# DISCOWER/fault-tolerant-mpc

Hardware: AMD Instinct MI355X
Metric: MPC QP steps/s (whole node) at N=20, 8 thrusters, batch 65536 (higher is better)
Workload: dtype f32

## Files before the change

fault-tolerant-mpc_amd/csrc/ftmpc_solve.hip:

```cpp
#include <hip/hip_runtime.h>

#include <type_traits>

#include "ftmpc_common.h"

namespace ftmpc {

namespace {

typedef float f32x4 __attribute__((ext_vector_type(4)));
typedef float f32x2 __attribute__((ext_vector_type(2)));

__device__ __forceinline__ void wave_lds_fence() { asm volatile("" ::: "memory"); }
__device__ __forceinline__ void wave_global_fence() { asm volatile("s_waitcnt vmcnt(0)" ::: "memory"); }
__device__ __forceinline__ int tidx(int I, int J) { return (I * (I + 1)) / 2 + J; }

__device__ __forceinline__ float readlane_f(float x, int l) {
    return __builtin_bit_cast(float, __builtin_amdgcn_readlane(__builtin_bit_cast(int, x), l));
}
struct OpAdd { static __device__ __forceinline__ float f(float a, float b) { return a + b; } };
struct OpMin { static __device__ __forceinline__ float f(float a, float b) { return fminf(a, b); } };
struct OpMax { static __device__ __forceinline__ float f(float a, float b) { return fmaxf(a, b); } };
template <class Op>
__device__ __forceinline__ float wave_reduce(float x) {
// ... 388 lines not shown
        {
            const f32x4 wj = Wof(J);
            float y0 = wj.x * r, y1 = wj.y * r, y2 = wj.z * r, y3 = wj.w * r;
            row_sum16x4(y0, y1, y2, y3);
            Y[J] = f32x4{y0, y1, y2, y3};
        }
#pragma unroll
        for (int I = J + 1; I < NB; ++I) {
            const f32x4& t = T[tidx(I, J)];
            p[I] += f32x2{t.x, t.y} * f32x2{Y[J].x, Y[J].y};
            p[I] += f32x2{t.z, t.w} * f32x2{Y[J].z, Y[J].w};
        }
    }
    wave_lds_fence();
    f32x2 a0[NB], a1[NB];
#pragma unroll
    for (int J = 0; J < NB; ++J) a0[J] = a1[J] = f32x2{0.f, 0.f};
    const int lb = lane_now();
    const int li_b = lb & 15, lq_b = lb >> 4;
#pragma unroll
    for (int J = NB - 1; J >= 0; --J) {
        f32x4 r = Y[J];
        if (J < NB - 1) {
            float s0 = a0[J].x, s1 = a0[J].y, s2 = a1[J].x, s3 = a1[J].y;
            row_sum16x4(s0, s1, s2, s3);
            r -= f32x4{s0, s1, s2, s3};
        }
        const f32x4 wb = Wof(J);
        const f32x2 d2 = f32x2{wb.x, wb.y} * f32x2{r.x, r.y} + f32x2{wb.z, wb.w} * f32x2{r.z, r.w};
        const float xr = quad_sum(d2.x + d2.y);
        if (lq_b == 0) xv[16 * J + li_b] = xr;
        const f32x2 xx = {xr, xr};
#pragma unroll
        for (int K = 0; K < J; ++K) {
            const f32x4& t = T[tidx(J, K)];
            a0[K] += f32x2{t.x, t.y} * xx;
            a1[K] += f32x2{t.z, t.w} * xx;
        }
    }
    wave_lds_fence();
}

__host__ __device__ constexpr int aoff(int r, int c) {
    constexpr int ZERO = REC_STRIDE, ONE = REC_STRIDE + 1, DT = REC_STRIDE + 2;
    if (r >= 13) return ZERO;
    const int kind = r < 3 ? 0 : (r < 6 ? 1 : (r < 9 ? 2 : 3));
    const int a = r < 3 ? r : (r < 6 ? r - 3 : (r < 9 ? r - 6 : r - 9));
    if (c < 3) return (kind == 0 && c == a) ? ONE : ZERO;
    if (c < 6) return (kind == 0 && c - 3 == a) ? DT : ((kind == 1 && c - 3 == a) ? ONE : ZERO);
    if (c < 9) {
        const int j = c - 6;
        return kind == 0 ? REC_APW + 3 * a + j : (kind == 1 ? REC_AVW + 3 * a + j : (kind == 2 ? REC_AWW + 3 * a + j : REC_AQW + 3 * a + j));
    }
    if (c < 13) {
        const int j = c - 9;
        return kind == 0 ? REC_APQ + 4 * a + j : (kind == 1 ? REC_AVQ + 4 * a + j : (kind == 2 ? ZERO : REC_AQQ + 4 * a + j));
    }
    if (c < 16) {
        const int j = c - 13;
        return kind == 0 ? REC_BPF + 3 * a + j : (kind == 1 ? REC_BVF + 3 * a + j : ZERO);
    }
    const int j = c - 16;
    return kind == 0 ? REC_BPT + 3 * a + j : (kind == 1 ? REC_BVT + 3 * a + j : (kind == 2 ? REC_BWT + 3 * a + j : REC_BQT + 3 * a + j));
}
struct AoffTable {
    unsigned char v[16][20];
};
constexpr AoffTable make_aoff_table() {
    AoffTable t{};
    for (int r = 0; r < 16; ++r)
        for (int c = 0; c < 20; ++c) t.v[r][c] = (unsigned char)((c < 19) ? aoff(r, c) : REC_STRIDE);
    return t;
}
__device__ const AoffTable k_aoff = make_aoff_table();
typedef double f64x4 __attribute__((ext_vector_type(4)));
__device__ __forceinline__ f64x4 mfma_d(double a, double b, f64x4 c) {
    return __builtin_amdgcn_mfma_f64_16x16x4f64(a, b, c, 0, 0, 0);
}

typedef __attribute__((address_space(3))) double lds_f64;
typedef __attribute__((address_space(3))) const float lds_cf32;
typedef __attribute__((address_space(1))) double glb_f64;
typedef __attribute__((address_space(1))) const double glb_cf64;
template <class SPtr, int GOFF = 160>
__device__ __noinline__ void struct_grad(const DeviceConsts& C, glb_cf64* recg, lds_f64* recd, lds_cf32* s_Da,
                                            lds_cf32* dnat, SPtr sS, glb_f64* gout, int na, int lane) {
    constexpr int ZERO = REC_STRIDE;
    const int N = C.N;
    const int m = lane & 15, q = lane >> 4;
    int offX[4], offG[2], offAT[4], offBT[4];
#pragma unroll
    for (int s4 = 0; s4 < 4; ++s4) {
        const int k = 4 * s4 + q;
        offX[s4] = (k < 13) ? k_aoff.v[m][k] : ZERO;
        offAT[s4] = (k < 13 && m < 13) ? k_aoff.v[k][m] : ZERO;
        offBT[s4] = (k < 13 && m < 6) ? k_aoff.v[k][13 + m] : ZERO;
    }
#pragma unroll
    for (int s4 = 0; s4 < 2; ++s4) offG[s4] = (4 * s4 + q < 6) ? k_aoff.v[m][13 + 4 * s4 + q] : ZERO;
    if (lane == 0) {
        recd[REC_STRIDE] = 0.0;
        recd[REC_STRIDE + 1] = 1.0;
        recd[REC_STRIDE + 2] = C.dt;
    }
    double qrow[4], rrow[2], da_op[2];
#pragma unroll
    for (int i = 0; i < 4; ++i) qrow[i] = (q + 4 * i < 9) ? C.Q[q + 4 * i] : 0.0;
#pragma unroll
    for (int i = 0; i < 2; ++i) {
        rrow[i] = (q + 4 * i < 6) ? C.R[q + 4 * i] : 0.0;
        da_op[i] = (q + 4 * i < 6) ? (double)s_Da[(q + 4 * i) * MAX_NT + m] : 0.0;
    }
    double pa[4];
#pragma unroll
    for (int s4 = 0; s4 < 4; ++s4) pa[s4] = (m < 9 && 4 * s4 + q < 9) ? C.P[9 * m + 4 * s4 + q] : 0.0;
    const f64x4 zero = {0.0, 0.0, 0.0, 0.0};
    glb_f64* genS = gout + GOFF;
    for (int t = lane; t < N * 8; t += 64) {
        const int k = t >> 3, g = t & 7;
        double acc = 0.0;
        if (g < 6)
            for (int a = 0; a < na; ++a) acc += (double)s_Da[g * MAX_NT + a] * (double)dnat[k * na + a];
        genS[t] = acc;
    }
    __threadfence_block();
    wave_global_fence();
    const int g1 = (q + 4 < 6) ? q + 4 : 7;
    double pf[4][3], pg[4][2];
    const int w2 = (lane + 128 < REC_STRIDE) ? lane + 128 : REC_STRIDE - 1;
    const int d2 = (lane + 128 < REC_STRIDE) ? lane + 128 : REC_STRIDE + 3;
    auto issue = [&](auto SL, int kk) {
        constexpr int sl = decltype(SL)::value;
        glb_cf64* r = recg + (int64_t)kk * REC_STRIDE;
        pf[sl][0] = r[lane];
        pf[sl][1] = r[lane + 64];
        pf[sl][2] = r[w2];
        pg[sl][0] = genS[kk * 8 + q];
        pg[sl][1] = genS[kk * 8 + g1];
    };
    auto stage_to_lds = [&](auto SL) {
        constexpr int sl = decltype(SL)::value;
        recd[lane] = pf[sl][0];
        recd[lane + 64] = pf[sl][1];
        recd[d2] = pf[sl][2];
    };
    using S0 = std::integral_constant<int, 0>;
    using S1 = std::integral_constant<int, 1>;
    using S2 = std::integral_constant<int, 2>;
    using S3 = std::integral_constant<int, 3>;
    f64x4 dc = zero;
    auto fwd = [&](auto SL, int k) {
        constexpr int sl = decltype(SL)::value;
        wave_lds_fence();
        stage_to_lds(SL);
        const double g0 = pg[sl][0], g1v = pg[sl][1];
        issue(SL, (k + 4 < N) ? k + 4 : N - 1);
        wave_lds_fence();
        f64x4 nx = zero, ny = zero;
        nx = mfma_d(recd[offX[0]], dc.x, nx);
        ny = mfma_d(recd[offX[1]], dc.y, ny);
        nx = mfma_d(recd[offX[2]], dc.z, nx);
        ny = mfma_d(recd[offX[3]], dc.w, ny);
        nx = mfma_d(recd[offG[0]], g0, nx);
        ny = mfma_d(recd[offG[1]], g1v, ny);
        dc = nx + ny;
        f64x4 t = zero;
        if (k + 1 == N) {
#pragma unroll
            for (int s4 = 0; s4 < 4; ++s4) t = mfma_d(pa[s4], dc[s4], t);
        } else {
#pragma unroll
            for (int i = 0; i < 3; ++i) t[i] = qrow[i] * dc[i];
        }
        if (m == 0) {
            SPtr srow = sS + (k + 1) * 9;
            srow[q] = recd[REC_WE + q] + t.x;
            srow[q + 4] = recd[REC_WE + q + 4] + t.y;
            if (q == 0) srow[8] = recd[REC_WE + 8] + t.z;
        }
    };
    const int N4 = N & ~3;
    issue(S0{}, 0);
    issue(S1{}, (1 < N) ? 1 : 0);
    issue(S2{}, (2 < N) ? 2 : 0);
    issue(S3{}, (3 < N) ? 3 : 0);
    for (int k = 0; k < N4; k += 4) {
        fwd(S0{}, k);
        fwd(S1{}, k + 1);
        fwd(S2{}, k + 2);
        fwd(S3{}, k + 3);
    }
    for (int k = N4; k < N; ++k) {
        issue(S0{}, k);
        fwd(S0{}, k);
    }
    wave_global_fence();
    f64x4 lam = zero;
    auto adj = [&](auto SL, int k) {
        constexpr int sl = decltype(SL)::value;
        wave_lds_fence();
        stage_to_lds(SL);
        const double g0 = pg[sl][0], g1v = pg[sl][1];
        issue(SL, (k - 4 >= 0) ? k - 4 : 0);
        wave_lds_fence();
        if (k == N - 1) {
            lam.x = sS[N * 9 + q];
            lam.y = sS[N * 9 + q + 4];
            lam.z = (q == 0) ? sS[N * 9 + 8] : 0.0;
            lam.w = 0.0;
        }
        f64x4 z = zero, zb = zero;
        z = mfma_d(recd[offBT[0]], lam.x, z);
        zb = mfma_d(recd[offBT[1]], lam.y, zb);
        z = mfma_d(recd[offBT[2]], lam.z, z);
        zb = mfma_d(recd[offBT[3]], lam.w, zb);
        z += zb;
        const double z0 = z.x + recd[REC_RUT + q] + rrow[0] * g0;
        const double z1 = (q + 4 < 6) ? z.y + recd[REC_RUT + q + 4] + rrow[1] * g1v : 0.0;
        f64x4 ga = zero;
        ga = mfma_d(da_op[0], z0, ga);
        ga = mfma_d(da_op[1], z1, ga);
        if (m == 0) {
#pragma unroll
            for (int i = 0; i < 4; ++i)
                if (q + 4 * i < na) gout[k * na + q + 4 * i] = 2.0 * ga[i];
        }
        if (k > 0) {
            f64x4 nl = zero, nm = zero;
            nl = mfma_d(recd[offAT[0]], lam.x, nl);
            nm = mfma_d(recd[offAT[1]], lam.y, nm);
            nl = mfma_d(recd[offAT[2]], lam.z, nl);
            nm = mfma_d(recd[offAT[3]], lam.w, nm);
            nl += nm;
            lam.x = nl.x + sS[k * 9 + q];
            lam.y = nl.y + sS[k * 9 + q + 4];
            lam.z = nl.z + ((q == 0) ? sS[k * 9 + 8] : 0.0);
            lam.w = nl.w;
        }
    };
    issue(S0{}, N - 1);
    issue(S1{}, (N - 2 >= 0) ? N - 2 : 0);
    issue(S2{}, (N - 3 >= 0) ? N - 3 : 0);
    issue(S3{}, (N - 4 >= 0) ? N - 4 : 0);
    int ka = N - 1;
    for (; ka >= 3; ka -= 4) {
        adj(S0{}, ka);
        adj(S1{}, ka - 1);
        adj(S2{}, ka - 2);
        adj(S3{}, ka - 3);
    }
    for (; ka >= 0; --ka) {
        issue(S0{}, ka);
        adj(S0{}, ka);
    }
    __threadfence_block();
    wave_global_fence();
}

__host__ __device__ constexpr int tile_row(int r) { return r < 9 ? 4 * (r % 3) + r / 3 : (r < 12 ? 12 + (r - 9) : 3); }
constexpr int DENSE_DUMP = 256 + 128;
constexpr int DENSE_WORDS = 400;
constexpr int dense_blk(int w, int base, int ncol, int rowc, int colc, bool isB) {
    const int a = (w - base) / ncol, c = (w - base) % ncol;
    return isB ? 256 + 8 * tile_row(rowc + a) + (colc + c) : 16 * tile_row(rowc + a) + tile_row(colc + c);
}
constexpr int dense_pos(int w) {
    if (w < REC_APQ) return dense_blk(w, REC_APW, 3, 0, 6, false);
    if (w < REC_AVW) return dense_blk(w, REC_APQ, 4, 0, 9, false);
    if (w < REC_AVQ) return dense_blk(w, REC_AVW, 3, 3, 6, false);
    if (w < REC_AWW) return dense_blk(w, REC_AVQ, 4, 3, 9, false);
    if (w < REC_AQW) return dense_blk(w, REC_AWW, 3, 6, 6, false);
    if (w < REC_AQQ) return dense_blk(w, REC_AQW, 3, 9, 6, false);
    if (w < REC_BPF) return dense_blk(w, REC_AQQ, 4, 9, 9, false);
    if (w < REC_BPT) return dense_blk(w, REC_BPF, 3, 0, 0, true);
    if (w < REC_BVF) return dense_blk(w, REC_BPT, 3, 0, 3, true);
    if (w < REC_BVT) return dense_blk(w, REC_BVF, 3, 3, 0, true);
    if (w < REC_BWT) return dense_blk(w, REC_BVT, 3, 3, 3, true);
    if (w < REC_BQT) return dense_blk(w, REC_BWT, 3, 6, 3, true);
    if (w < REC_WE) return dense_blk(w, REC_BQT, 3, 9, 3, true);
    return DENSE_DUMP;
}
struct DensePosTable {
    unsigned short v[REC_STRIDE];
};
constexpr DensePosTable make_dense_pos() {
    DensePosTable t{};
    for (int w = 0; w < REC_STRIDE; ++w) t.v[w] = (unsigned short)dense_pos(w);
    return t;
}
__device__ const DensePosTable k_dense_pos = make_dense_pos();
constexpr bool dense_pos_ok() {
    bool used[DENSE_WORDS] = {};
    for (int a = 0; a < 3; ++a) {
        used[16 * tile_row(a) + tile_row(a)] = true;
        used[16 * tile_row(a) + tile_row(3 + a)] = true;
        used[16 * tile_row(3 + a) + tile_row(3 + a)] = true;
    }
    for (int w = 0; w < REC_STRIDE; ++w) {
        const int p = dense_pos(w);
        if (w >= REC_WE) {
            if (p != DENSE_DUMP) return false;
            continue;
        }
        if (p < 0 || p >= DENSE_DUMP || used[p]) return false;
        used[p] = true;
    }
    return true;
}
static_assert(dense_pos_ok(), "stage-record scatter table is inconsistent");
constexpr bool tile_row_ok() {
    bool seen[16] = {};
    for (int r = 0; r < 13; ++r) {
        const int t = tile_row(r);
        if (t < 0 || t > 15 || seen[t]) return false;
        seen[t] = true;
        if (r < 9 && ((t & 3) > 2 || (t >> 2) > 2)) return false;
    }
    return true;
}
static_assert(tile_row_ok(), "state-component permutation of the sensitivity tiles is inconsistent");

}

#ifndef FTMPC_F32_MU_POLISH
#define FTMPC_F32_MU_POLISH 1e-5f
#endif
#ifndef FTMPC_F32_REFINE_AT_POLISH
#define FTMPC_F32_REFINE_AT_POLISH 1
#endif
#ifndef FTMPC_F32_REGRAD_DD
#define FTMPC_F32_REGRAD_DD 2e-4f
#endif
#ifndef FTMPC_F32_PW0
#define FTMPC_F32_PW0 1e3f
#endif
#ifndef FTMPC_F32_OCC
#define FTMPC_F32_OCC 2
#endif
template <int NB>
__global__ void __launch_bounds__(64) __attribute__((amdgpu_waves_per_eu((NB == 8) ? FTMPC_F32_OCC : 1, (NB == 8) ? FTMPC_F32_OCC : 1))) ftmpc_solve_f32_kernel(const DeviceConsts C, const SolveParams P) {
    using SH = Shape<NB>;
    constexpr int NPAD = SH::NPAD, NV = SH::NV, NTILES = SH::NTILES;
    constexpr int NLDS = (NB == 8) ? ((FTMPC_F32_OCC > 1) ? 0 : NTILES) : (NB == 9 ? 36 : 35);
    constexpr bool OCC2 = (NB == 8) && (FTMPC_F32_OCC > 1);
    constexpr int BUILD_WORDS = 2 * DENSE_WORDS + 256;
    __shared__ __attribute__((aligned(16))) float tiles[(NLDS * 256 > BUILD_WORDS) ? NLDS * 256 : BUILD_WORDS];
    __shared__ __attribute__((aligned(16))) float recbuf[2 * REC_STRIDE + 8];
    __shared__ __attribute__((aligned(16))) float work[SH::WORK + SH::SEXTRA];
    __shared__ __attribute__((aligned(16))) float s_Da[6 * MAX_NT];
    __shared__ unsigned char s_stg[NPAD], s_thr[NPAD];
    __shared__ int s_act[MAX_NT];
    __shared__ __attribute__((aligned(16))) float wlds[OCC2 ? NB * 256 : 4];
    float* const dense = tiles;
    float* const xvp = work;
    float* const dvp = work + NPAD;

    const int lane = threadIdx.x;
    const int li = lane & 15, lq = lane >> 4;
    const int N = C.N, NT = C.NT;
    TileStore<NLDS> htiles;
    htiles.p = tiles;
    htiles.bind(P.hscratch + (int64_t)blockIdx.x * P.tile_words + slot_tile_off_words(C.N));
    const float rho = (float)C.rho;
    const float mu_stop = (float)C.mu_stop;
    float Rf[6];
#pragma unroll
    for (int g = 0; g < 6; ++g) Rf[g] = (float)C.R[g];

    auto pull = [&]() {
        int i = 0;
        if (lane == 0) i = atomicAdd(P.qhead, 1);
        return i;
    };
    const int qn = *P.qcount;
    int qnext = pull();
    for (;;) {
        const int qi = __builtin_amdgcn_readfirstlane(qnext);
        if (qi >= qn) break;
        const int64_t inst = P.qlist[qi];
        qnext = pull();
        STAMP_DECL;
        STAMP_START();
        wave_lds_fence();
        double ub_l = 0.0;
        if (lane < NT) ub_l = P.ub[inst * NT + lane];
        const unsigned long long amask = __ballot(lane < NT && ub_l > 0.0);
        const int na = __popcll(amask);
        const int n = N * na;
        const int nb = (n + 15) >> 4;
        const int npad = nb * 16;
        (void)npad;
        if (na == 0 || nb > NB) {
            if (lane < NT) P.out_u0[inst * NT + lane] = 0.0;
            if (P.out_U)
                for (int i = lane; i < N * NT; i += 64) P.out_U[inst * N * NT + i] = 0.0;
            if (lane == 0) {
                if (P.status) P.status[inst] = (na == 0) ? 0 : 2;
                if (P.iters) P.iters[inst] = 0;
            }
            continue;
        }
        const int nbr = NB;
        const int npadr = 16 * nbr;
        const int myrank = __popcll(amask & ((1ull << lane) - 1ull));
        if (lane < NT && ub_l > 0.0) s_act[myrank] = lane;
        wave_lds_fence();
        if (lane < na) {
#pragma unroll
            for (int g = 0; g < 6; ++g) s_Da[g * MAX_NT + lane] = (float)C.D[g * MAX_NT + s_act[lane]];
        }
        for (int e = lane; e < npadr; e += 64) {
            const int s = e / na;
            s_stg[e] = (unsigned char)(e < n ? s : 255);
            s_thr[e] = (unsigned char)(e < n ? e - s * na : 255);
        }
        typedef double f64x4_t __attribute__((ext_vector_type(4)));
        const double* recg = reinterpret_cast<const double*>(P.rec) + inst * (int64_t)N * REC_STRIDE;
        f64x4_t pre64 = {0.0, 0.0, 0.0, 0.0};
        if (lane < REC_STRIDE / 4) pre64 = *reinterpret_cast<const f64x4_t*>(recg + 4 * lane);
        int dpos[4] = {DENSE_DUMP, DENSE_DUMP, DENSE_DUMP, DENSE_DUMP};
        {
            int w0 = 4 * lane;
            asm volatile("" : "+v"(w0));
            if (lane < REC_STRIDE / 4) {
                const ushort4 t = *reinterpret_cast<const ushort4*>(&k_dense_pos.v[w0]);
                dpos[0] = t.x;
                dpos[1] = t.y;
                dpos[2] = t.z;
                dpos[3] = t.w;
            }
        }
        for (int i = lane; i < 2 * DENSE_WORDS + 256; i += 64) dense[i] = 0.f;
        wave_lds_fence();
        if (lane < 6) {
            const int a = lane % 3, isv = lane / 3;
#pragma unroll
            for (int bsel = 0; bsel < 2; ++bsel) {
                float* dd = dense + bsel * DENSE_WORDS;
                dd[16 * tile_row(3 * isv + a) + tile_row(3 * isv + a)] = 1.f;
                if (!isv) dd[16 * tile_row(a) + tile_row(3 + a)] = (float)C.dt;
            }
        }
        for (int i = lane; i < 81; i += 64) {
            const int r = i / 9, c = i - 9 * r;
            if (c >= r) dense[2 * DENSE_WORDS + 16 * tile_row(r) + tile_row(c)] = (float)C.LPt[i];
        }
        wave_lds_fence();
        const f32x4 lp4 = lds4(dense + 2 * DENSE_WORDS + 16 * li + 4 * lq);

        int kcol[NV], acol[NV];
        float ubar[NV], ubv[NV], gacc[NV];
#pragma unroll
        for (int v = 0; v < NV; ++v) {
            const int e = v * 64 + lane;
            kcol[v] = (e < npadr) ? s_stg[e] : 255;
            acol[v] = (e < npadr) ? s_thr[e] : 255;
            ubar[v] = 0.f;
            ubv[v] = 1.f;
            gacc[v] = 0.f;
            if (kcol[v] != 255) {
                const int t = s_act[acol[v]];
                ubv[v] = (float)P.ub[inst * NT + t];
                if (P.warmU) {
                    const float wv = (float)P.warmU[(inst * N + kcol[v]) * NT + t];
                    ubar[v] = fminf(fmaxf(wv, 0.f), ubv[v]);
                }
            }
        }
        int kX[OCC2 ? 1 : NB];
        float DaB[OCC2 ? 1 : NB][2];
        f32x4 G[NB];
        float gpart[NB];
#pragma unroll
        for (int X = 0; X < NB; ++X) {
            if constexpr (!OCC2) {
                kX[X] = s_stg[16 * X + li];
                const int ax = s_thr[16 * X + li];
                DaB[X][0] = (ax != 255) ? s_Da[lq * MAX_NT + ax] : 0.f;
                DaB[X][1] = (ax != 255 && lq < 2) ? s_Da[(4 + lq) * MAX_NT + ax] : 0.f;
            }
            G[X] = (f32x4){0.f, 0.f, 0.f, 0.f};
            gpart[X] = 0.f;
        }
        float esc[3];
#pragma unroll
        for (int s3 = 0; s3 < 3; ++s3) esc[s3] = (lq < 3) ? (OCC2 ? 2.f * (float)C.Q[3 * s3 + lq] : (float)C.sq2Q[3 * s3 + lq]) : 0.f;
        f32x4 acc[NTILES];
#pragma unroll
        for (int t = 0; t < NTILES; ++t) acc[t] = (f32x4){0.f, 0.f, 0.f, 0.f};

        float* const mtab = work;
        auto finish_tile = [&](int I, int J) {
            const int lane = lane_now();
            const int li = lane & 15, lq = lane >> 4;
            f32x4 h = acc[(I * (I + 1)) / 2 + J];
            if (J >= I - 1) {
#pragma unroll
                for (int rr = 0; rr < 4; ++rr) {
                    const int e1 = (I == J) ? 16 * I + 4 * lq + rr : 16 * I + li;
                    const int e2 = (I == J) ? 16 * J + li : 16 * J + 4 * lq + rr;
                    const int s1 = s_stg[e1], a1 = s_thr[e1];
                    const int s2 = s_stg[e2], a2 = s_thr[e2];
                    float add = (s1 != 255 && s1 == s2) ? mtab[((a1 & (MAX_NT - 1)) << 4) | (a2 & (MAX_NT - 1))] : 0.f;
                    if (s1 == 255 && e1 == e2) add = 1.f;
                    h[rr] += add;
                }
            }
            htiles.st((I * (I + 1)) / 2 + J, lane, -h);
        };

        STAMP(0);
        auto stage = [&](int k, auto TERM) {
            constexpr bool terminal = decltype(TERM)::value;
            const int lane = lane_now();
            const int li = lane & 15, lq = lane >> 4;
            float* rb = recbuf + (k & 1) * REC_STRIDE;
            float* dd = dense + (k & 1) * DENSE_WORDS;
            if (lane < REC_STRIDE / 4) {
                const f32x4 pre = {(float)pre64.x, (float)pre64.y, (float)pre64.z, (float)pre64.w};
                *reinterpret_cast<f32x4*>(rb + 4 * lane) = pre;
                dd[dpos[0]] = pre.x;
                dd[dpos[1]] = pre.y;
                dd[dpos[2]] = pre.z;
                dd[dpos[3]] = pre.w;
                if (!terminal) pre64 = *reinterpret_cast<const f64x4_t*>(recg + (k + 1) * REC_STRIDE + 4 * lane);
            }
            wave_lds_fence();
            const f32x4 a4 = lds4(dd + 16 * li + 4 * lq);
            const float b0 = dd[256 + 8 * li + lq], b1 = dd[256 + 8 * li + 4 + lq];
            float we[3];
#pragma unroll
            for (int s3 = 0; s3 < 3; ++s3) we[s3] = (lq < 3) ? rb[REC_WE + 3 * s3 + lq] : 0.f;
            const float rut0 = rb[REC_RUT + lq], rut1 = (lq < 2) ? rb[REC_RUT + 4 + lq] : 0.f;
            const int Imax = ((k + 1) * na - 1) >> 4;
            const int Xnew = (k * na) >> 4;
            float E[NB][3];
            const f32x4 zero4 = {0.f, 0.f, 0.f, 0.f};
#pragma unroll
            for (int X = 0; X < NB; ++X)
                if (X <= Imax) {
                    f32x4 o = zero4;
                    if (X >= Xnew) {
                        float d0, d1;
                        if constexpr (OCC2) {
                            const int ax = *(lds_vu8*)&s_thr[16 * X + li];
                            const bool mine = (*(lds_vu8*)&s_stg[16 * X + li] == k);
                            d0 = mine ? s_Da[lq * MAX_NT + (ax & (MAX_NT - 1))] : 0.f;
                            d1 = (mine && lq < 2) ? s_Da[(4 + lq) * MAX_NT + (ax & (MAX_NT - 1))] : 0.f;
                        } else {
                            const bool mine = (kX[X] == k);
                            d0 = mine ? DaB[X][0] : 0.f;
                            d1 = mine ? DaB[X][1] : 0.f;
                        }
                        o = mfma4(b0, d0, o);
                        o = mfma4(b1, d1, o);
                        gpart[X] += d0 * rut0 + d1 * rut1;
                    }
                    o = mfma4(a4.x, G[X].x, o);
                    o = mfma4(a4.y, G[X].y, o);
                    o = mfma4(a4.z, G[X].z, o);
                    o = mfma4(a4.w, G[X].w, o);
                    G[X] = o;
                }
#pragma unroll
            for (int X = 0; X < NB; ++X)
                if (X <= Imax) {
                    gpart[X] += we[0] * G[X].x + we[1] * G[X].y + we[2] * G[X].z;
                    if (!terminal) {
                        if constexpr (!OCC2) {
                            E[X][0] = esc[0] * G[X].x;
                            E[X][1] = esc[1] * G[X].y;
                            E[X][2] = esc[2] * G[X].z;
                        }
                    } else {
                        f32x4 o = zero4;
                        o = mfma4(lp4.x, G[X].x, o);
                        o = mfma4(lp4.y, G[X].y, o);
                        o = mfma4(lp4.z, G[X].z, o);
                        o = mfma4(lp4.w, G[X].w, o);
                        E[X][0] = o.x;
                        E[X][1] = o.y;
                        E[X][2] = o.z;
                    }
                }
            STAMP(1);
#pragma unroll
            for (int I = 0; I < NB; ++I)
                if (I <= Imax) {
                    float eI[3] = {0.f, 0.f, 0.f};
                    if constexpr (OCC2 && !terminal) {
                        eI[0] = esc[0] * G[I].x;
                        eI[1] = esc[1] * G[I].y;
                        eI[2] = esc[2] * G[I].z;
                    }
#pragma unroll
                    for (int J = 0; J <= I; ++J) {
                        if constexpr (OCC2 && !terminal) {
                            acc[(I * (I + 1)) / 2 + J] = mfma4(G[J].x, eI[0], acc[(I * (I + 1)) / 2 + J]);
                            acc[(I * (I + 1)) / 2 + J] = mfma4(G[J].y, eI[1], acc[(I * (I + 1)) / 2 + J]);
                            acc[(I * (I + 1)) / 2 + J] = mfma4(G[J].z, eI[2], acc[(I * (I + 1)) / 2 + J]);
                        } else {
#pragma unroll
                        for (int s3 = 0; s3 < 3; ++s3) acc[(I * (I + 1)) / 2 + J] = mfma4(E[J][s3], E[I][s3], acc[(I * (I + 1)) / 2 + J]);
                        }
                        if constexpr (terminal) finish_tile(I, J);
                    }
                }
            STAMP(2);
        };
        for (int k = 0; k + 1 < N; ++k) stage(k, std::false_type{});
        for (int t = lane; t < MAX_NT * MAX_NT; t += 64) {
            const int a1 = t >> 4, a2 = t & (MAX_NT - 1);
            float m = 0.f;
            if (a1 < na && a2 < na) {
#pragma unroll
                for (int g = 0; g < 6; ++g) m += s_Da[g * MAX_NT + a1] * Rf[g] * s_Da[g * MAX_NT + a2];
                if (a1 == a2) m += rho;
            }
            mtab[t] = 2.f * m;
        }
        wave_lds_fence();
        stage(N - 1, std::true_type{});
#pragma unroll
        for (int I = 0; I < NB; ++I)
            if (I > ((N * na - 1) >> 4)) {
#pragma unroll
                for (int J = 0; J <= I; ++J) finish_tile(I, J);
            }
        {
            float qs[NB];
#pragma unroll
            for (int X = 0; X < NB; ++X) qs[X] = quad_sum(gpart[X]);
#pragma unroll
            for (int v = 0; v < NV; ++v) {
                float t = 0.f;
#pragma unroll
                for (int j = 0; j < 4; ++j)
                    if (4 * v + j < NB) t = (lq == j) ? qs[4 * v + j] : t;
                gacc[v] += t;
            }
        }
        wave_lds_fence();

        float gv[NV], lo[NV], hi[NV], sl[NV], su[NV], zl[NV], zu[NV], grad[NV];
        bool valid[NV];
#pragma unroll
        for (int v = 0; v < NV; ++v) {
            valid[v] = kcol[v] != 255;
            gv[v] = valid[v] ? 2.f * (gacc[v] + rho * ubar[v]) : 0.f;
            lo[v] = -ubar[v];
            hi[v] = ubv[v] - ubar[v];
            sl[v] = su[v] = 0.5f * ubv[v];
        }
        if (P.dbg_inst == inst) {
#pragma unroll
            for (int I = 0; I < NB; ++I)
                if (I < nbr) {
#pragma unroll
                    for (int J = 0; J <= I; ++J) {
                        const f32x4 ht = htiles.ld((I * (I + 1)) / 2 + J, lane);
#pragma unroll
                        for (int rr = 0; rr < 4; ++rr) {
                            const int e1 = (I == J) ? 16 * I + 4 * lq + rr : 16 * I + li;
                            const int e2 = (I == J) ? 16 * J + li : 16 * J + 4 * lq + rr;
                            const float h = -ht[rr];
                            if (I != J || e1 >= e2) {
                                P.dbg_H[(int64_t)e1 * npadr + e2] = h;
                                P.dbg_H[(int64_t)e2 * npadr + e1] = h;
                            }
                        }
                    }
                }
#pragma unroll
            for (int v = 0; v < NV; ++v) {
                const int e = v * 64 + lane;
                if (e < npadr) {
                    P.dbg_vec[e] = gv[v];
                    P.dbg_vec[npadr + e] = lo[v];
                    P.dbg_vec[2 * npadr + e] = hi[v];
                }
            }
            if (lane == 0) {
                P.dbg_vec[480] = (float)n;
                P.dbg_vec[481] = (float)npadr;
            }
        }

        STAMP(3);
        f32x4 Tt[NTILES], Wd[NB];
        int status = 1, nit = 0;
        bool first = true;
        double gref[NV];
        float dref[NV];
        bool refined = !(C.mu_refine > 0.0);
        float mu_last = 3.0e38f;
        double* const sbuf = reinterpret_cast<double*>(P.hscratch + (int64_t)blockIdx.x * P.tile_words);
#pragma unroll
        for (int v = 0; v < NV; ++v) {
            gref[v] = (double)gv[v];
            dref[v] = 0.f;
        }
        const float inv2n = 1.0f / (float)(2 * n);
        int pol = 0;
        bool pol_tried = !(FTMPC_F32_MU_POLISH > 0.f);
        bool pol_grad = false;
        unsigned pact = 0u;
        float pw = 0.f;
        float* const bkp = P.hscratch + (int64_t)blockIdx.x * P.tile_words + slot_backup_off_words(N);
        for (int it = 0; it <= C.max_iters; ++it) {
            wave_lds_fence();
            const int lane = lane_now();
            const int li = lane & 15, lq = lane >> 4;
            (void)li; (void)lq;
            const bool do_ref = __builtin_amdgcn_readfirstlane(!refined && mu_last < (float)C.mu_refine && (pol_tried || !FTMPC_F32_REFINE_AT_POLISH));
            float dcur[NV];
            if (it == 0) {
#pragma unroll
                for (int v = 0; v < NV; ++v) dcur[v] = valid[v] ? ((sl[v] < su[v]) ? lo[v] + sl[v] : hi[v] - su[v]) : 0.f;
            }
            auto refresh = [&]() {
                float dnow[NV];
#pragma unroll
                for (int v = 0; v < NV; ++v) {
                    dnow[v] = valid[v] ? ((sl[v] < su[v]) ? lo[v] + sl[v] : hi[v] - su[v]) : 0.f;
                    const int e = v * 64 + lane;
                    if (e < npadr) xvp[e] = dnow[v];
                }
                wave_lds_fence();
                constexpr int SAVAIL = (NPAD + SH::SEXTRA) * 4;
                double* const gout = sbuf;
                if ((N + 1) * 72 <= SAVAIL)
                    struct_grad(C, (glb_cf64*)recg, (lds_f64*)reinterpret_cast<double*>(recbuf), (lds_cf32*)s_Da, (lds_cf32*)xvp,
                                (lds_f64*)reinterpret_cast<double*>(dvp), (glb_f64*)gout, na, lane);
                else
                    struct_grad(C, (glb_cf64*)recg, (lds_f64*)reinterpret_cast<double*>(recbuf), (lds_cf32*)s_Da, (lds_cf32*)xvp,
                                (glb_f64*)(sbuf + slot_stage_off(N)), (glb_f64*)gout, na, lane);
#pragma unroll
                for (int v = 0; v < NV; ++v) {
                    const int e = v * 64 + lane;
                    gref[v] = (valid[v] && e < n) ? gout[e] + 2.0 * C.rho * ((double)ubar[v] + (double)dnow[v]) : 0.0;
                    dref[v] = dnow[v];
                    grad[v] = valid[v] ? (float)gref[v] : 0.f;
                }
                refined = true;
                STAMP(8);
            };
            if (do_ref) {
                refresh();
            } else if (it == 0) {
#pragma unroll
            for (int v = 0; v < NV; ++v) {
                const int e = v * 64 + lane;
                if (e < npadr) dvp[e] = dcur[v] - dref[v];
            }
            wave_lds_fence();
            {
                f32x2 arow[NB];
                f32x4 acol[NB];
#pragma unroll
                for (int I = 0; I < NB; ++I) {
                    arow[I] = f32x2{0.f, 0.f};
                    acol[I] = f32x4{0.f, 0.f, 0.f, 0.f};
                }
#pragma unroll
                for (int I = 0; I < NB; ++I) {
                    const float dI = dvp[16 * I + li];
#pragma unroll
                    for (int J = 0; J <= I; ++J) {
                        const f32x4 t4 = htiles.ld((I * (I + 1)) / 2 + J, lane);
                        const f32x4 d4 = lds4(dvp + 16 * J + 4 * lq);
                        arow[I] += f32x2{t4.x, t4.y} * f32x2{d4.x, d4.y};
                        arow[I] += f32x2{t4.z, t4.w} * f32x2{d4.z, d4.w};
                        if (J < I) acol[J] += t4 * dI;
                    }
                }
                wave_lds_fence();
#pragma unroll
                for (int J = 0; J < NB; ++J) {
                    float c0 = acol[J].x, c1 = acol[J].y, c2 = acol[J].z, c3 = acol[J].w;
                    row_sum16x4(c0, c1, c2, c3);
                    const f32x4 c4 = {c0, c1, c2, c3};
                    if (li == 0) *reinterpret_cast<f32x4*>(xvp + 16 * J + 4 * lq) = c4;
                }
                wave_lds_fence();
                float yrow[NB];
#pragma unroll
                for (int I = 0; I < NB; ++I) yrow[I] = quad_sum(arow[I].x + arow[I].y);
#pragma unroll
                for (int v = 0; v < NV; ++v) {
                    float t = 0.f;
#pragma unroll
                    for (int j = 0; j < 4; ++j)
                        if (4 * v + j < NB) t = (lq == j) ? yrow[4 * v + j] : t;
                    const int e = v * 64 + lane;
                    const float hd = -(t + ((e < npadr) ? xvp[e] : 0.f));
                    grad[v] = valid[v] ? (float)((double)hd + gref[v]) : 0.f;
                }
                wave_lds_fence();
            }
            }
            STAMP(4);
            float t = 0.f;
            if (first) {
                float gm = 0.f, wm = 0.f;
#pragma unroll
                for (int v = 0; v < NV; ++v)
                    if (valid[v]) {
                        gm = fmaxf(gm, fabsf(grad[v]));
                        wm = fmaxf(wm, ubv[v]);
                    }
                gm = wave_max(gm);
                wm = wave_max(wm);
                const float mu0 = fmaxf(0.02f * gm * wm, 1e-3f);
#pragma unroll
                for (int v = 0; v < NV; ++v) {
                    zl[v] = valid[v] ? mu0 / sl[v] : 0.f;
                    zu[v] = valid[v] ? mu0 / su[v] : 0.f;
                }
                first = false;
            }
#pragma unroll
            for (int v = 0; v < NV; ++v)
                if (valid[v]) t += sl[v] * zl[v] + su[v] * zu[v];
            const float mu = wave_sum(t) * inv2n;
            mu_last = mu;
            if (__builtin_amdgcn_readfirstlane(!pol && !(mu >= mu_stop))) {
                status = (mu == mu) ? 0 : 2;
                break;
            }
            if (it == C.max_iters) break;
            ++nit;
            if (__builtin_amdgcn_readfirstlane(!pol && !pol_tried && mu < FTMPC_F32_MU_POLISH)) {
                pol_tried = true;
                pol = 1;
                float hs = 0.f;
#pragma unroll
                for (int I = 0; I < NB; ++I) {
                    const f32x4 t4 = htiles.ld((I * (I + 1)) / 2 + I, lane);
                    const int r = li - 4 * lq;
                    const float dg = (r == 0) ? t4.x : (r == 1) ? t4.y : (r == 2) ? t4.z : t4.w;
                    if (r >= 0 && r < 4 && 16 * I + li < n) hs = fmaxf(hs, -dg);
                }
                pw = FTMPC_F32_PW0 * wave_max(hs);
                pact = 0u;
#pragma unroll
                for (int v = 0; v < NV; ++v) {
                    bkp[(0 * NV + v) * 64 + lane] = sl[v];
                    bkp[(1 * NV + v) * 64 + lane] = su[v];
                    bkp[(2 * NV + v) * 64 + lane] = zl[v];
                    bkp[(3 * NV + v) * 64 + lane] = zu[v];
                    bkp[(4 * NV + v) * 64 + lane] = grad[v];
                    const bool al = valid[v] && zl[v] > sl[v], au = valid[v] && zu[v] > su[v];
                    pact |= (al ? 1u : 0u) << (2 * v) | (au ? 2u : 0u) << (2 * v);
                    zl[v] = al ? zl[v] : 0.f;
                    zu[v] = au ? zu[v] : 0.f;
                }
            }
            auto pol_abandon = [&]() {
#pragma unroll
                for (int v = 0; v < NV; ++v) {
                    sl[v] = bkp[(0 * NV + v) * 64 + lane];
                    su[v] = bkp[(1 * NV + v) * 64 + lane];
                    zl[v] = bkp[(2 * NV + v) * 64 + lane];
                    zu[v] = bkp[(3 * NV + v) * 64 + lane];
                    grad[v] = bkp[(4 * NV + v) * 64 + lane];
                }
                pol = 0;
                refined = false;
            };
            auto pol_rhs = [&](int v) -> float {
                float r = 0.f;
                if (valid[v]) {
                    r = -grad[v];
                    if (pact >> (2 * v) & 1u) r -= pw * sl[v] - zl[v];
                    if (pact >> (2 * v + 1) & 1u) r += pw * su[v] - zu[v];
                }
                return r;
            };
            auto pol_signs = [&]() -> bool {
                bool changed = false;
#pragma unroll
                for (int v = 0; v < NV; ++v)
                    if (valid[v]) {
                        const unsigned bl = 1u << (2 * v), bu = 2u << (2 * v);
                        if (pact & bl) {
                            if (zl[v] < 0.f) { zl[v] = 0.f; pact &= ~bl; changed = true; }
                        } else if (sl[v] < -1e-6f * ubv[v]) { pact |= bl; changed = true; }
                        if (pact & bu) {
                            if (zu[v] < 0.f) { zu[v] = 0.f; pact &= ~bu; changed = true; }
                        } else if (su[v] < -1e-6f * ubv[v]) { pact |= bu; changed = true; }
                    }
                return __any(changed);
            };
            auto pol_step = [&](int v, float r, float dd) {
                if (valid[v]) {
                    const bool al = pact >> (2 * v) & 1u, au = pact >> (2 * v + 1) & 1u;
                    grad[v] += r - ((al ? pw : 0.f) + (au ? pw : 0.f)) * dd;
                    if (al) zl[v] += pw * (-dd - sl[v]);
                    if (au) zu[v] += pw * (dd - su[v]);
                    sl[v] += dd;
                    su[v] -= dd;
                }
            };
            f32x4 pre0[NB];
            chol_prefetch_col0<NB>(htiles, lane, pre0);
            float Sig[NV], rsl[NV], rsu[NV];
            wave_lds_fence();
#pragma unroll
            for (int v = 0; v < NV; ++v) {
                rsl[v] = __builtin_amdgcn_rcpf(sl[v]);
                rsu[v] = __builtin_amdgcn_rcpf(su[v]);
                Sig[v] = valid[v] ? zl[v] * rsl[v] + zu[v] * rsu[v] : 0.f;
                if (pol) Sig[v] = ((pact >> (2 * v) & 1u) ? pw : 0.f) + ((pact >> (2 * v + 1) & 1u) ? pw : 0.f);
                const int e = v * 64 + lane;
                if (e < npadr) dvp[e] = Sig[v];
            }
            wave_lds_fence();
            STAMP(7);
            const bool ok = chol_reg<NB, TileStore<NLDS>, true, OCC2>(htiles, dvp, recbuf, n, lane, Tt, Wd, pre0, wlds);
            STAMP(5);
            if (__builtin_amdgcn_readfirstlane(!ok)) {
                if (pol) {
                    pol_abandon();
                    continue;
                }
                status = 2;
                break;
            }
            float rcl[NV], rcu[NV], rhs[NV];
#pragma unroll
            for (int v = 0; v < NV; ++v) {
                const int e = v * 64 + lane;
                rhs[v] = pol ? pol_rhs(v) : -grad[v];
                if (e < npadr) xvp[e] = rhs[v];
            }
            wave_lds_fence();
            STAMP(7);
            solve_reg<NB, OCC2>(Tt, Wd, xvp, nbr, lane, wlds);
            STAMP(6);
            float da[NV], dzl_a[NV], dzu_a[NV];
            float ap = 1.f, ad = 1.f;
#pragma unroll
            for (int v = 0; v < NV; ++v) {
                const int e = v * 64 + lane;
                da[v] = (e < npadr && valid[v]) ? xvp[e] : 0.f;
                dzl_a[v] = dzu_a[v] = 0.f;
                if (pol) {
                    pol_step(v, rhs[v], da[v]);
                } else if (valid[v]) {
                    dzl_a[v] = -zl[v] - zl[v] * da[v] * rsl[v];
                    dzu_a[v] = -zu[v] + zu[v] * da[v] * rsu[v];
                    const float rda = __builtin_amdgcn_rcpf(da[v]);
                    if (da[v] < 0.f) ap = fminf(ap, -sl[v] * rda);
                    if (da[v] > 0.f) ap = fminf(ap, su[v] * rda);
                    if (dzl_a[v] < 0.f) ad = fminf(ad, -zl[v] * __builtin_amdgcn_rcpf(dzl_a[v]));
                    if (dzu_a[v] < 0.f) ad = fminf(ad, -zu[v] * __builtin_amdgcn_rcpf(dzu_a[v]));
                }
            }
            bool regrad = false;
            if (pol) {
                if (pol_signs()) {
                    if (++pol > 3) pol_abandon();
                    continue;
                }
                regrad = !pol_grad;
                if (!regrad) {
                    float ddm = 0.f;
#pragma unroll
                    for (int v = 0; v < NV; ++v)
                        if (valid[v]) ddm = fmaxf(ddm, fabsf(da[v]) * __builtin_amdgcn_rcpf(ubv[v]));
                    regrad = wave_max(ddm) > FTMPC_F32_REGRAD_DD;
                }
                pol_grad = true;
            }
            if (regrad) {
                typedef __attribute__((address_space(1))) f32x4 glb_f32x4;
                glb_f32x4* const fpark = (glb_f32x4*)(P.hscratch + (int64_t)blockIdx.x * P.tile_words + slot_factor_off_words(N));
                int slotn = 0;
#pragma unroll
                for (int I = 1; I < NB; ++I)
#pragma unroll
                    for (int J = 0; J < I; ++J) fpark[(slotn++) * 64 + lane] = Tt[tidx(I, J)];
                if constexpr (!OCC2) {
#pragma unroll
                    for (int J = 0; J < NB; ++J) fpark[(slotn++) * 64 + lane] = Wd[J];
                }
                refresh();
                slotn = 0;
#pragma unroll
                for (int I = 1; I < NB; ++I)
#pragma unroll
                    for (int J = 0; J < I; ++J) Tt[tidx(I, J)] = fpark[(slotn++) * 64 + lane];
                if constexpr (!OCC2) {
#pragma unroll
                    for (int J = 0; J < NB; ++J) Wd[J] = fpark[(slotn++) * 64 + lane];
                }
            }
            ap = wave_min(ap);
            ad = wave_min(ad);
            t = 0.f;
#pragma unroll
            for (int v = 0; v < NV; ++v)
                if (valid[v]) t += (sl[v] + ap * da[v]) * (zl[v] + ad * dzl_a[v]) + (su[v] - ap * da[v]) * (zu[v] + ad * dzu_a[v]);
            const float mu_aff = wave_sum(t) * inv2n;
            float sigma = mu_aff / mu;
            sigma = fminf(fmaxf(sigma * sigma * sigma, 0.f), 1.f);
            wave_lds_fence();
#pragma unroll
            for (int v = 0; v < NV; ++v) {
                rcl[v] = rcu[v] = rhs[v] = 0.f;
                if (pol) {
                    rhs[v] = pol_rhs(v);
                } else if (valid[v]) {
                    rcl[v] = sl[v] * zl[v] + da[v] * dzl_a[v] - sigma * mu;
                    rcu[v] = su[v] * zu[v] - da[v] * dzu_a[v] - sigma * mu;
                    rhs[v] = -(grad[v] - zl[v] + zu[v]) - rcl[v] * rsl[v] + rcu[v] * rsu[v];
                }
                const int e = v * 64 + lane;
                if (e < npadr) xvp[e] = rhs[v];
            }
            wave_lds_fence();
            STAMP(7);
            solve_reg<NB, OCC2>(Tt, Wd, xvp, nbr, lane, wlds);
            STAMP(6);
            float dd[NV], dzl[NV], dzu[NV];
            ap = 1e30f;
            ad = 1e30f;
            if (pol) {
#pragma unroll
                for (int v = 0; v < NV; ++v) {
                    const int e = v * 64 + lane;
                    pol_step(v, rhs[v], (e < npadr && valid[v]) ? xvp[e] : 0.f);
                }
                const bool changed = pol_signs();
                STAMP(7);
                if (!changed) {
                    status = 0;
                    break;
                }
                if (++pol > 3) pol_abandon();
                continue;
            }
#pragma unroll
            for (int v = 0; v < NV; ++v) {
                const int e = v * 64 + lane;
                dd[v] = (e < npadr && valid[v]) ? xvp[e] : 0.f;
                dzl[v] = dzu[v] = 0.f;
                if (valid[v]) {
                    dzl[v] = (-rcl[v] - zl[v] * dd[v]) * rsl[v];
                    dzu[v] = (-rcu[v] + zu[v] * dd[v]) * rsu[v];
                    const float rdd = __builtin_amdgcn_rcpf(dd[v]);
                    if (dd[v] < 0.f) ap = fminf(ap, -sl[v] * rdd);
                    if (dd[v] > 0.f) ap = fminf(ap, su[v] * rdd);
                    if (dzl[v] < 0.f) ad = fminf(ad, -zl[v] * __builtin_amdgcn_rcpf(dzl[v]));
                    if (dzu[v] < 0.f) ad = fminf(ad, -zu[v] * __builtin_amdgcn_rcpf(dzu[v]));
                }
            }
            ap = fminf(1.f, 0.9995f * wave_min(ap));
            ad = fminf(1.f, 0.9995f * wave_min(ad));
#pragma unroll
            for (int v = 0; v < NV; ++v)
                if (valid[v]) {
                    grad[v] += ap * (rhs[v] - Sig[v] * dd[v]);
                    sl[v] += ap * dd[v];
                    su[v] -= ap * dd[v];
                    zl[v] += ad * dzl[v];
                    zu[v] += ad * dzu[v];
                }
            STAMP(7);
        }

        wave_lds_fence();
        float* ubuf = tiles;
        for (int i = lane; i < N * NT; i += 64) ubuf[i] = 0.f;
        wave_lds_fence();
#pragma unroll
        for (int v = 0; v < NV; ++v)
            if (valid[v]) {
                float u = fminf(fmaxf((sl[v] < su[v]) ? sl[v] : ubv[v] - su[v], 0.f), ubv[v]);
// ... 27 lines not shown
```

Baseline: 5.028 million.

## Move struct_grad exchange to LDS, read constants from kernarg/LDS, hand off prefetches

Generalizes struct_grad so the gradient buffer and stage buffer can live in LDS, using cheap LDS fences instead of global fences in the OCC2 path. Constants are read from the kernarg segment or an LDS copy rather than through the DeviceConsts reference. Record prefetches are issued before the gradient precompute, and forward-pass prefetches are handed off directly to the adjoint pass when N is a multiple of 4. It also precomputes the polish diagonal max during Hessian assembly, and overlaps unparking the factor tiles with the tail of refresh. Gains come from fewer global memory round trips and less latency, at the cost of more code complexity and extra LDS use.

```diff
diff --git a/fault-tolerant-mpc_amd/csrc/ftmpc_solve.hip b/fault-tolerant-mpc_amd/csrc/ftmpc_solve.hip
--- a/fault-tolerant-mpc_amd/csrc/ftmpc_solve.hip
+++ b/fault-tolerant-mpc_amd/csrc/ftmpc_solve.hip
@@ -494,11 +494,26 @@
 typedef __attribute__((address_space(3))) const float lds_cf32;
 typedef __attribute__((address_space(1))) double glb_f64;
 typedef __attribute__((address_space(1))) const double glb_cf64;
-template <class SPtr, int GOFF = 160>
-__device__ __noinline__ void struct_grad(const DeviceConsts& C, glb_cf64* recg, lds_f64* recd, lds_cf32* s_Da,
-                                            lds_cf32* dnat, SPtr sS, glb_f64* gout, int na, int lane) {
+typedef __attribute__((address_space(3))) const double lds_cf64;
+typedef __attribute__((address_space(4))) const double karg_cf64;
+constexpr int CT_D = 0, CT_Q = CT_D + 6 * MAX_NT, CT_R = CT_Q + 9, CT_P = CT_R + 6, CT_LPT = CT_P + 81, CT_SQ2Q = CT_LPT + 81, CT_WORDS = CT_SQ2Q + 9;
+static_assert(offsetof(DeviceConsts, Q) == offsetof(DeviceConsts, D) + 8 * CT_Q && offsetof(DeviceConsts, R) == offsetof(DeviceConsts, D) + 8 * CT_R &&
+              offsetof(DeviceConsts, P) == offsetof(DeviceConsts, D) + 8 * CT_P && offsetof(DeviceConsts, LPt) == offsetof(DeviceConsts, D) + 8 * CT_LPT &&
+              offsetof(DeviceConsts, sq2Q) == offsetof(DeviceConsts, D) + 8 * CT_SQ2Q && offsetof(DeviceConsts, rho) == offsetof(DeviceConsts, D) + 8 * CT_WORDS,
+              "the constant table is the run D .. sq2Q of DeviceConsts");
+template <class SPtr, class GPtr, class CPtr, int GOFF = 160>
+__device__ __noinline__ void struct_grad_at(int N, double dt, CPtr ctab, glb_cf64* recg, lds_f64* recd, lds_cf32* s_Da,
+                                            lds_cf32* dnat, SPtr sS, GPtr gout, int na, int lane) {
     constexpr int ZERO = REC_STRIDE;
-    const int N = C.N;
+    constexpr bool GLOBAL_XCHG = std::is_same<SPtr, glb_f64*>::value || std::is_same<GPtr, glb_f64*>::value;
+    auto xchg_fence = [&]() {
+        if constexpr (GLOBAL_XCHG) {
+            __threadfence_block();
+            wave_global_fence();
+        } else {
+            wave_lds_fence();
+        }
+    };
     const int m = lane & 15, q = lane >> 4;
     int offX[4], offG[2], offAT[4], offBT[4];
 #pragma unroll
@@ -513,42 +528,40 @@
     if (lane == 0) {
         recd[REC_STRIDE] = 0.0;
         recd[REC_STRIDE + 1] = 1.0;
-        recd[REC_STRIDE + 2] = C.dt;
+        recd[REC_STRIDE + 2] = dt;
     }
     double qrow[4], rrow[2], da_op[2];
 #pragma unroll
-    for (int i = 0; i < 4; ++i) qrow[i] = (q + 4 * i < 9) ? C.Q[q + 4 * i] : 0.0;
+    for (int i = 0; i < 4; ++i) qrow[i] = (q + 4 * i < 9) ? ctab[CT_Q + q + 4 * i] : 0.0;
 #pragma unroll
     for (int i = 0; i < 2; ++i) {
-        rrow[i] = (q + 4 * i < 6) ? C.R[q + 4 * i] : 0.0;
+        rrow[i] = (q + 4 * i < 6) ? ctab[CT_R + q + 4 * i] : 0.0;
         da_op[i] = (q + 4 * i < 6) ? (double)s_Da[(q + 4 * i) * MAX_NT + m] : 0.0;
     }
     double pa[4];
 #pragma unroll
-    for (int s4 = 0; s4 < 4; ++s4) pa[s4] = (m < 9 && 4 * s4 + q < 9) ? C.P[9 * m + 4 * s4 + q] : 0.0;
+    for (int s4 = 0; s4 < 4; ++s4) pa[s4] = (m < 9 && 4 * s4 + q < 9) ? ctab[CT_P + 9 * m + 4 * s4 + q] : 0.0;
     const f64x4 zero = {0.0, 0.0, 0.0, 0.0};
-    glb_f64* genS = gout + GOFF;
-    for (int t = lane; t < N * 8; t += 64) {
-        const int k = t >> 3, g = t & 7;
-        double acc = 0.0;
-        if (g < 6)
-            for (int a = 0; a < na; ++a) acc += (double)s_Da[g * MAX_NT + a] * (double)dnat[k * na + a];
-        genS[t] = acc;
-    }
-    __threadfence_block();
-    wave_global_fence();
     const int g1 = (q + 4 < 6) ? q + 4 : 7;
+    GPtr genS = gout + GOFF;
     double pf[4][3], pg[4][2];
     const int w2 = (lane + 128 < REC_STRIDE) ? lane + 128 : REC_STRIDE - 1;
     const int d2 = (lane + 128 < REC_STRIDE) ? lane + 128 : REC_STRIDE + 3;
-    auto issue = [&](auto SL, int kk) {
+    auto issue_rec = [&](auto SL, int kk) {
         constexpr int sl = decltype(SL)::value;
         glb_cf64* r = recg + (int64_t)kk * REC_STRIDE;
         pf[sl][0] = r[lane];
         pf[sl][1] = r[lane + 64];
         pf[sl][2] = r[w2];
+    };
+    auto issue_gen = [&](auto SL, int kk) {
+        constexpr int sl = decltype(SL)::value;
         pg[sl][0] = genS[kk * 8 + q];
         pg[sl][1] = genS[kk * 8 + g1];
+    };
+    auto issue = [&](auto SL, int kk) {
+        issue_rec(SL, kk);
+        issue_gen(SL, kk);
     };
     auto stage_to_lds = [&](auto SL) {
         constexpr int sl = decltype(SL)::value;
@@ -560,13 +573,27 @@
     using S1 = std::integral_constant<int, 1>;
     using S2 = std::integral_constant<int, 2>;
     using S3 = std::integral_constant<int, 3>;
+    const int N4 = N & ~3;
+    issue_rec(S0{}, 0);
+    issue_rec(S1{}, (1 < N) ? 1 : 0);
+    issue_rec(S2{}, (2 < N) ? 2 : 0);
+    issue_rec(S3{}, (3 < N) ? 3 : 0);
+    for (int t = lane; t < N * 8; t += 64) {
+        const int k = t >> 3, g = t & 7;
+        double acc = 0.0;
+        if (g < 6)
+            for (int a = 0; a < na; ++a) acc += (double)s_Da[g * MAX_NT + a] * (double)dnat[k * na + a];
+        genS[t] = acc;
+    }
+    xchg_fence();
+    const bool hand_on = N4 == N;
     f64x4 dc = zero;
     auto fwd = [&](auto SL, int k) {
         constexpr int sl = decltype(SL)::value;
         wave_lds_fence();
         stage_to_lds(SL);
         const double g0 = pg[sl][0], g1v = pg[sl][1];
-        issue(SL, (k + 4 < N) ? k + 4 : N - 1);
+        issue(SL, (k + 4 < N) ? k + 4 : (hand_on ? 2 * N - 5 - k : N - 1));
         wave_lds_fence();
         f64x4 nx = zero, ny = zero;
         nx = mfma_d(recd[offX[0]], dc.x, nx);
@@ -584,18 +611,19 @@
 #pragma unroll
             for (int i = 0; i < 3; ++i) t[i] = qrow[i] * dc[i];
         }
+        double s0 = recd[REC_WE + q] + t.x, s1 = recd[REC_WE + q + 4] + t.y, s2 = recd[REC_WE + 8] + t.z;
+        asm volatile("" : "+v"(s0), "+v"(s1), "+v"(s2));
         if (m == 0) {
             SPtr srow = sS + (k + 1) * 9;
-            srow[q] = recd[REC_WE + q] + t.x;
-            srow[q + 4] = recd[REC_WE + q + 4] + t.y;
-            if (q == 0) srow[8] = recd[REC_WE + 8] + t.z;
+            srow[q] = s0;
+            srow[q + 4] = s1;
+            if (q == 0) srow[8] = s2;
         }
     };
-    const int N4 = N & ~3;
-    issue(S0{}, 0);
-    issue(S1{}, (1 < N) ? 1 : 0);
-    issue(S2{}, (2 < N) ? 2 : 0);
-    issue(S3{}, (3 < N) ? 3 : 0);
+    issue_gen(S0{}, 0);
+    issue_gen(S1{}, (1 < N) ? 1 : 0);
+    issue_gen(S2{}, (2 < N) ? 2 : 0);
+    issue_gen(S3{}, (3 < N) ? 3 : 0);
     for (int k = 0; k < N4; k += 4) {
         fwd(S0{}, k);
         fwd(S1{}, k + 1);
@@ -606,7 +634,8 @@
         issue(S0{}, k);
         fwd(S0{}, k);
     }
-    wave_global_fence();
+    if constexpr (std::is_same<SPtr, glb_f64*>::value) wave_global_fence();
+    else wave_lds_fence();
     f64x4 lam = zero;
     auto adj = [&](auto SL, int k) {
         constexpr int sl = decltype(SL)::value;
@@ -650,10 +679,12 @@
             lam.w = nl.w;
         }
     };
-    issue(S0{}, N - 1);
-    issue(S1{}, (N - 2 >= 0) ? N - 2 : 0);
-    issue(S2{}, (N - 3 >= 0) ? N - 3 : 0);
-    issue(S3{}, (N - 4 >= 0) ? N - 4 : 0);
+    if (!hand_on) {
+        issue(S0{}, N - 1);
+        issue(S1{}, (N - 2 >= 0) ? N - 2 : 0);
+        issue(S2{}, (N - 3 >= 0) ? N - 3 : 0);
+        issue(S3{}, (N - 4 >= 0) ? N - 4 : 0);
+    }
     int ka = N - 1;
     for (; ka >= 3; ka -= 4) {
         adj(S0{}, ka);
@@ -665,8 +696,13 @@
         issue(S0{}, ka);
         adj(S0{}, ka);
     }
-    __threadfence_block();
-    wave_global_fence();
+    xchg_fence();
+}
+
+template <class SPtr, int GOFF = 160>
+__device__ __forceinline__ void struct_grad(const DeviceConsts& C, glb_cf64* recg, lds_f64* recd, lds_cf32* s_Da,
+                                            lds_cf32* dnat, SPtr sS, glb_f64* gout, int na, int lane) {
+    struct_grad_at<SPtr, glb_f64*, const double*, GOFF>(C.N, C.dt, &C.D[0], recg, recd, s_Da, dnat, sS, gout, na, lane);
 }
 
 __host__ __device__ constexpr int tile_row(int r) { return r < 9 ? 4 * (r % 3) + r / 3 : (r < 12 ? 12 + (r - 9) : 3); }
@@ -762,6 +798,18 @@
     __shared__ __attribute__((aligned(16))) float s_Da[6 * MAX_NT];
     __shared__ unsigned char s_stg[NPAD], s_thr[NPAD];
     __shared__ int s_act[MAX_NT];
+    constexpr bool CLDS = OCC2;
+    karg_cf64* const kctab = (karg_cf64*)((__attribute__((address_space(4))) const char*)__builtin_amdgcn_kernarg_segment_ptr() + offsetof(DeviceConsts, D));
+    using CPtr = typename std::conditional<CLDS, lds_cf64*, karg_cf64*>::type;
+    CPtr ctab;
+    if constexpr (CLDS) {
+        __shared__ double s_ctab[CT_WORDS];
+        for (int i = threadIdx.x; i < CT_WORDS; i += 64) s_ctab[i] = kctab[i];
+        wave_lds_fence();
+        ctab = (lds_cf64*)s_ctab;
+    } else {
+        ctab = kctab;
+    }
     __shared__ __attribute__((aligned(16))) float wlds[OCC2 ? NB * 256 : 4];
     float* const dense = tiles;
     float* const xvp = work;
@@ -794,6 +842,8 @@
         STAMP_DECL;
         STAMP_START();
         wave_lds_fence();
+        const int lane = lane_now();
+        const int li = lane & 15, lq = lane >> 4;
         double ub_l = 0.0;
         if (lane < NT) ub_l = P.ub[inst * NT + lane];
         const unsigned long long amask = __ballot(lane < NT && ub_l > 0.0);
@@ -819,7 +869,7 @@
         wave_lds_fence();
         if (lane < na) {
 #pragma unroll
-            for (int g = 0; g < 6; ++g) s_Da[g * MAX_NT + lane] = (float)C.D[g * MAX_NT + s_act[lane]];
+            for (int g = 0; g < 6; ++g) s_Da[g * MAX_NT + lane] = (float)ctab[CT_D + g * MAX_NT + s_act[lane]];
         }
         for (int e = lane; e < npadr; e += 64) {
             const int s = e / na;
@@ -855,7 +905,7 @@
         }
         for (int i = lane; i < 81; i += 64) {
             const int r = i / 9, c = i - 9 * r;
-            if (c >= r) dense[2 * DENSE_WORDS + 16 * tile_row(r) + tile_row(c)] = (float)C.LPt[i];
+            if (c >= r) dense[2 * DENSE_WORDS + 16 * tile_row(r) + tile_row(c)] = (float)ctab[CT_LPT + i];
         }
         wave_lds_fence();
         const f32x4 lp4 = lds4(dense + 2 * DENSE_WORDS + 16 * li + 4 * lq);
@@ -896,12 +946,13 @@
         }
         float esc[3];
 #pragma unroll
-        for (int s3 = 0; s3 < 3; ++s3) esc[s3] = (lq < 3) ? (OCC2 ? 2.f * (float)C.Q[3 * s3 + lq] : (float)C.sq2Q[3 * s3 + lq]) : 0.f;
+        for (int s3 = 0; s3 < 3; ++s3) esc[s3] = (lq < 3) ? (OCC2 ? 2.f * (float)ctab[CT_Q + 3 * s3 + lq] : (float)ctab[CT_SQ2Q + 3 * s3 + lq]) : 0.f;
         f32x4 acc[NTILES];
 #pragma unroll
         for (int t = 0; t < NTILES; ++t) acc[t] = (f32x4){0.f, 0.f, 0.f, 0.f};
 
         float* const mtab = work;
+        float hdmax = 0.f;
         auto finish_tile = [&](int I, int J) {
             const int lane = lane_now();
             const int li = lane & 15, lq = lane >> 4;
@@ -917,6 +968,11 @@
                     if (s1 == 255 && e1 == e2) add = 1.f;
                     h[rr] += add;
                 }
+            }
+            if (I == J) {
+                const int r = li - 4 * lq;
+                const float dg = (r == 0) ? h.x : (r == 1) ? h.y : (r == 2) ? h.z : h.w;
+                if (r >= 0 && r < 4 && 16 * I + li < n) hdmax = fmaxf(hdmax, dg);
             }
             htiles.st((I * (I + 1)) / 2 + J, lane, -h);
         };
@@ -1053,6 +1109,7 @@
             }
         }
         wave_lds_fence();
+        const float pw_diag = __builtin_bit_cast(float, __builtin_amdgcn_readfirstlane(__builtin_bit_cast(int, FTMPC_F32_PW0 * wave_max(hdmax))));
 
         float gv[NV], lo[NV], hi[NV], sl[NV], su[NV], zl[NV], zu[NV], grad[NV];
         bool valid[NV];
@@ -1130,7 +1187,7 @@
 #pragma unroll
                 for (int v = 0; v < NV; ++v) dcur[v] = valid[v] ? ((sl[v] < su[v]) ? lo[v] + sl[v] : hi[v] - su[v]) : 0.f;
             }
-            auto refresh = [&]() {
+            auto refresh = [&](auto between) {
                 float dnow[NV];
 #pragma unroll
                 for (int v = 0; v < NV; ++v) {
@@ -1141,16 +1198,27 @@
                 wave_lds_fence();
                 constexpr int SAVAIL = (NPAD + SH::SEXTRA) * 4;
                 double* const gout = sbuf;
-                if ((N + 1) * 72 <= SAVAIL)
-                    struct_grad(C, (glb_cf64*)recg, (lds_f64*)reinterpret_cast<double*>(recbuf), (lds_cf32*)s_Da, (lds_cf32*)xvp,
-                                (lds_f64*)reinterpret_cast<double*>(dvp), (glb_f64*)gout, na, lane);
-                else
-                    struct_grad(C, (glb_cf64*)recg, (lds_f64*)reinterpret_cast<double*>(recbuf), (lds_cf32*)s_Da, (lds_cf32*)xvp,
+                constexpr bool GLDS = OCC2;
+                static_assert(!GLDS || (160 + 8 * (SAVAIL / 72 - 1)) * 2 <= BUILD_WORDS, "gradient and wrench perturbations beyond the tile area");
+                lds_f64* const gout_l = (lds_f64*)reinterpret_cast<double*>(tiles);
+                const bool s_in_lds = (N + 1) * 72 <= SAVAIL;
+                if (s_in_lds) {
+                    if constexpr (GLDS)
+                        struct_grad_at(N, C.dt, ctab, (glb_cf64*)recg, (lds_f64*)reinterpret_cast<double*>(recbuf), (lds_cf32*)s_Da, (lds_cf32*)xvp,
+                                    (lds_f64*)reinterpret_cast<double*>(dvp), gout_l, na, lane);
+                    else
+                        struct_grad_at(N, C.dt, ctab, (glb_cf64*)recg, (lds_f64*)reinterpret_cast<double*>(recbuf), (lds_cf32*)s_Da, (lds_cf32*)xvp,
+                                    (lds_f64*)reinterpret_cast<double*>(dvp), (glb_f64*)gout, na, lane);
+                } else
+                    struct_grad_at(N, C.dt, ctab, (glb_cf64*)recg, (lds_f64*)reinterpret_cast<double*>(recbuf), (lds_cf32*)s_Da, (lds_cf32*)xvp,
                                 (glb_f64*)(sbuf + slot_stage_off(N)), (glb_f64*)gout, na, lane);
+                between();
 #pragma unroll
                 for (int v = 0; v < NV; ++v) {
                     const int e = v * 64 + lane;
-                    gref[v] = (valid[v] && e < n) ? gout[e] + 2.0 * C.rho * ((double)ubar[v] + (double)dnow[v]) : 0.0;
+                    double ge = 0.0;
+                    if (valid[v] && e < n) ge = (GLDS && s_in_lds) ? (double)gout_l[e] : gout[e];
+                    gref[v] = (valid[v] && e < n) ? ge + 2.0 * C.rho * ((double)ubar[v] + (double)dnow[v]) : 0.0;
                     dref[v] = dnow[v];
                     grad[v] = valid[v] ? (float)gref[v] : 0.f;
                 }
@@ -1158,7 +1226,7 @@
                 STAMP(8);
             };
             if (do_ref) {
-                refresh();
+                refresh([] {});
             } else if (it == 0) {
 #pragma unroll
             for (int v = 0; v < NV; ++v) {
@@ -1245,15 +1313,7 @@
             if (__builtin_amdgcn_readfirstlane(!pol && !pol_tried && mu < FTMPC_F32_MU_POLISH)) {
                 pol_tried = true;
                 pol = 1;
-                float hs = 0.f;
-#pragma unroll
-                for (int I = 0; I < NB; ++I) {
-                    const f32x4 t4 = htiles.ld((I * (I + 1)) / 2 + I, lane);
-                    const int r = li - 4 * lq;
-                    const float dg = (r == 0) ? t4.x : (r == 1) ? t4.y : (r == 2) ? t4.z : t4.w;
-                    if (r >= 0 && r < 4 && 16 * I + li < n) hs = fmaxf(hs, -dg);
-                }
-                pw = FTMPC_F32_PW0 * wave_max(hs);
+                pw = pw_diag;
                 pact = 0u;
 #pragma unroll
                 for (int v = 0; v < NV; ++v) {
@@ -1397,16 +1457,18 @@
 #pragma unroll
                     for (int J = 0; J < NB; ++J) fpark[(slotn++) * 64 + lane] = Wd[J];
                 }
-                refresh();
-                slotn = 0;
-#pragma unroll
-                for (int I = 1; I < NB; ++I)
-#pragma unroll
-                    for (int J = 0; J < I; ++J) Tt[tidx(I, J)] = fpark[(slotn++) * 64 + lane];
-                if constexpr (!OCC2) {
-#pragma unroll
-                    for (int J = 0; J < NB; ++J) Wd[J] = fpark[(slotn++) * 64 + lane];
-                }
+                auto unpark = [&]() {
+                    int slotr = 0;
+#pragma unroll
+                    for (int I = 1; I < NB; ++I)
+#pragma unroll
+                        for (int J = 0; J < I; ++J) Tt[tidx(I, J)] = fpark[(slotr++) * 64 + lane];
+                    if constexpr (!OCC2) {
+#pragma unroll
+                        for (int J = 0; J < NB; ++J) Wd[J] = fpark[(slotr++) * 64 + lane];
+                    }
+                };
+                refresh(unpark);
             }
             ap = wave_min(ap);
             ad = wave_min(ad);
```

After: 5.480 million (median of 6 runs). 1.09x the previous value.
